# chhylp123/BitMapperBS

Hardware: NVIDIA B200
Metric: mapped_reads_per_sec (higher is better)
Workload: dtype u64

## Files before the change

bitmapperbs_b200/csrc/bmbs_kernels.cuh:

```cuda
#pragma once
#include "bmbs_device.cuh"
#include "bmbs_sort_replay.h"
#include "bmbs_band_walk.h"
#include "../../include/bmbs.h"

namespace bmbs {

constexpr int MAX_TASKS = 28;
constexpr u32 MAX_SEED_HITS = 1000;
constexpr u32 MAX_PE_MULTI = 10000;
constexpr u32 MAX_PE_MULTI_SENSITIVE = 10000;

struct SeedTask { u64 sp; u32 hits; unsigned short mlen, off; };

enum { CNT_HASH = 0, CNT_OCC = 1, CNT_ROWS = 2, CNT_LOCATE_LF = 3, CNT_VERIFIED = 4, CNT_CELLS = 5, CNT_CAND = 6, CNT_WINBYTES = 7 };

struct __align__(16) VerifyItem { u64 site; u32 wi, vote, code_off, L, k, pad; };

struct BatchView {
  const char* ascii; const u64* offsets; int n_reads; int pe;
  u32* codes; uint4* rplanes; u32* len; unsigned short* first_c; unsigned char* kk;
  unsigned char* state; unsigned char* flags;
  short* one_mm; u64* site0;
  u32* list_count;
// ... 40 lines not shown
    const u32 cb = b0 | (b1 << 1) | (bad << 2);
    nib = (cb & 0xFu) | ((cb >> 4) & 0xF0u) | ((cb >> 8) & 0xF00u) | ((cb >> 12) & 0xF000u);
    o.bad = gather4(bad); o.isn = gather4(isn);
  }
  o.nib = nib; o.lo = gather4(b0); o.hi = gather4(b1);
  return o;
}

__device__ __forceinline__ u32 spread8(u32 v) {
  u32 t = (v * 0x1001u) & 0x000F000Fu;
  t = (t * 0x41u) & 0x03030303u;
  return (t * 9u) & 0x11111111u;
}
__device__ __forceinline__ bool pack8(u32 x0, u32 x1, u32& nib, u32& lo8, u32& hi8) {
  const u32 a1 = x0 >> 1, a2 = x0 >> 2, c1 = x1 >> 1, c2 = x1 >> 2;
  const u32 l0 = (a1 ^ a2) & 0x01010101u, h0 = a2 & 0x01010101u, l1 = (c1 ^ c2) & 0x01010101u, h1 = c2 & 0x01010101u;
  lo8 = ((l1 * 16u + l0) * 0x01020408u) >> 24;
  hi8 = ((h1 * 16u + h0) * 0x01020408u) >> 24;
  nib = spread8(hi8) * 2u + spread8(lo8);
  const u32 d0 = x0 ^ __byte_perm(0x54474341u, 0u, nib), d1 = x1 ^ __byte_perm(0x54474341u, 0u, nib >> 16);
  return (d0 | d1) == 0;
}

__global__ void __launch_bounds__(128) pack_reads(BatchView b) {
  const int r = (blockIdx.x * blockDim.x + threadIdx.x) >> 3, sub = threadIdx.x & 7;
  const bool live = r < b.n_reads;
  u64 beg = 0; u32 L = 0;
  if (live) { beg = b.offsets[r]; L = (u32)(b.offsets[r + 1] - beg); }
  u32* w = b.codes + (live ? code_word_offset(b.offsets, r) : 0);
  uint4* pl = b.rplanes + (live ? plane_chunk_offset(b.offsets, r) : 0);
  u32 first_c = L;
  for (u32 c = sub; c * 32 < L; c += 8) {
    const u64 addr = (u64)(b.ascii) + beg + (u64)c * 32;
    const u64* q = (const u64*)(addr & ~7ull);
    const unsigned sh = (unsigned)(addr & 7ull) * 8;
    u64 x[5];
#pragma unroll
    for (int i = 0; i < 5; ++i) x[i] = __ldg(q + i);
    if (sh) {
#pragma unroll
      for (int i = 0; i < 4; ++i) x[i] = (x[i] >> sh) | (x[i + 1] << (64 - sh));
    }
    const u32 left = L - c * 32;
    u32 lo = 0, hi = 0, bad = 0, isn = 0;
    u32 nw[4] = {0u, 0u, 0u, 0u};
#pragma unroll
    for (int i = 0; i < 4; ++i) {
      const u32 base = 8 * i;
      u32 n8, l8, h8;
      if (base < left && pack8((u32)x[i], (u32)(x[i] >> 32), n8, l8, h8)) {
        const u32 nb = left - base;
        if (nb < 8) { n8 &= (1u << (4 * nb)) - 1u; l8 &= (1u << nb) - 1u; h8 &= (1u << nb) - 1u; }
        nw[i] = n8;
        lo |= l8 << base; hi |= h8 << base;
      } else if (base < left) {
        const Packed4 a = pack4((u32)x[i], left - base);
        const Packed4 d = pack4((u32)(x[i] >> 32), left > base + 4 ? left - base - 4 : 0);
        nw[i] = a.nib | (d.nib << 16);
        lo |= (a.lo | (d.lo << 4)) << base; hi |= (a.hi | (d.hi << 4)) << base;
        bad |= (a.bad | (d.bad << 4)) << base; isn |= (a.isn | (d.isn << 4)) << base;
      }
    }
    *reinterpret_cast<uint4*>(w + c * 4) = make_uint4(nw[0], nw[1], nw[2], nw[3]);
    pl[c] = make_uint4(lo, hi, bad, isn);
    const u32 isc = lo & ~hi & ~bad;
    if (isc) first_c = min(first_c, c * 32 + (u32)__ffs(isc) - 1u);
  }
  for (int o = 4; o; o >>= 1) first_c = min(first_c, __shfl_xor_sync(0xffffffffu, first_c, o));
  if (live && sub == 0) {
    b.len[r] = L;
    b.first_c[r] = (unsigned short)first_c;
    u64 k = (u64)(b.e_rate * (double)L);
    b.kk[r] = (unsigned char)(k >= 31 ? 31 : k);
  }
}

struct SeedHit { u64 hits, sp, ep; u32 mlen; bool has_sa; u64 sa; };

constexpr int SEED_BLOCK = 128;
struct ReadPlanes {
  const uint4* p; const uint4* s; u32 ns;
  __device__ __forceinline__ void stage(const uint4* src, u32 L, uint4* smem_col, u32 cap) {
    p = src; s = smem_col;
    ns = (L >> 5) + 2; if (ns > cap) ns = cap;
    for (u32 i = 0; i < ns; ++i) smem_col[i * SEED_BLOCK] = __ldg(src + i);
  }
  __device__ __forceinline__ uint4 chunk(u32 i) const { return i < ns ? s[i * SEED_BLOCK] : __ldg(p + i); }
  __device__ __forceinline__ void window(u32 pos, u32& lo, u32& hi, u32& bad) const {
    const uint4 a = chunk(pos >> 5), c = chunk((pos >> 5) + 1);
    const unsigned s = pos & 31u;
    lo = __funnelshift_r(a.x, c.x, s); hi = __funnelshift_r(a.y, c.y, s); bad = __funnelshift_r(a.z, c.z, s);
  }
};

__device__ __forceinline__ bool key16(const ReadPlanes& rp, const unsigned char* __restrict__ lut, u32 off, u32& key) {
  u32 lo, hi, bad; rp.window(off, lo, hi, bad);
  if (bad & 0xFFFFu) return false;
  const u32 a = (lo & 0xFFFFu) | ((~lo & ~hi) << 16);
  const u32 i0 = (a & 0xFu) | ((a >> 12) & 0xF0u), i1 = ((a >> 4) & 0xFu) | ((a >> 16) & 0xF0u);
  const u32 i2 = ((a >> 8) & 0xFu) | ((a >> 20) & 0xF0u), i3 = ((a >> 12) & 0xFu) | ((a >> 24) & 0xF0u);
  key = (u32)lut[i0] + 81u * (u32)lut[i1] + 6561u * (u32)lut[i2] + 531441u * (u32)lut[i3];
  return true;
}

struct SymbolStream {
  const ReadPlanes& rp; u32 base, lo, hi, bad;
  __device__ __forceinline__ SymbolStream(const ReadPlanes& r, u32 pos, u32 l, u32 h, u32 b) : rp(r), base(pos), lo(l), hi(h), bad(b) {}
  __device__ __forceinline__ int at(u32 pos) {
    if (pos - base >= 32u) { base = pos; rp.window(pos, lo, hi, bad); }
    const unsigned s = pos - base;
    if ((bad >> s) & 1u) return 3;
    const u32 l = (lo >> s) & 1u, h = (hi >> s) & 1u;
    return (int)(l | ((~(l | h) & 1u) << 1));
  }
};

__device__ __forceinline__ bool kmer_ext(const DevIndex& ix, const unsigned char* __restrict__ lut, u32 lo, u32 hi, u32 bad, u32& ext) {
  const u32 mask = (1u << ix.kdepth) - 1u;
  if (bad & mask) return false;
  ext = lut[(lo & mask) | (((~lo & ~hi) & mask) << 4)];
  return true;
}

enum { START_NONE = 0, START_ANSWER = 1, START_LF = 2 };
__device__ __forceinline__ int seed_start(const DevIndex& ix, const ReadPlanes& rp, const unsigned char* lut, u32 off, u32 cur, bool exact,
                                          u32& m, u64& top, u64& bot, bool& one_sa, u32& lo, u32& hi, u32& bad, u32& n_hash) {
  int how = START_LF;
  u32 key;
  one_sa = false;
  if (cur < (exact ? 17u : 18u) || !key16(rp, lut, off, key)) how = START_NONE;
  else {
    m = 16;
    rp.window(off + 16, lo, hi, bad);
    bool in_table = false;
    if (ix.ktab && cur >= 16 + ix.kdepth) {
      u32 ext;
      if (kmer_ext(ix, lut, lo, hi, bad, ext)) {
        const u64 e = __ldg(ix.ktab + (u64)key * ix.kpow + ext); ++n_hash;
        const u64 size = e >> 39; const u32 code = (u32)(e >> 36) & 7u;
        if (size != KTAB_SAT) {
          in_table = true;
          if (code == 0) how = START_NONE;
          else {
            m = 15 + code; top = e & 0xFFFFFFFFFull; bot = top + size; one_sa = size == 1;
            const bool stops_short = m < 16 + ix.kdepth;
            if (!exact) { if (one_sa || stops_short) how = START_ANSWER; }
            else if (stops_short && size >= 2) how = START_NONE;
          }
        }
      }
    }
    if (!in_table) {
      hash_query(ix, key, top, bot); ++n_hash;
      if (bot <= top) how = START_NONE;
    }
  }
  if (how == START_NONE) { m = 0; top = 0; bot = 0; one_sa = false; }
  return how;
}

__device__ __forceinline__ bool exact_tail_matches(const DevIndex& ix, const ReadPlanes& rp, u64 s0, u32 off, u32 from, u32 cur) {
  if (s0 + cur > 2 * ix.N) return false;
  for (u32 p = off + from; p < off + cur; p += 32) {
    u32 rlo, rhi, rbad; rp.window(p, rlo, rhi, rbad);
    const u64 g = s0 + (p - off);
    const uint2 w0 = __ldg(ix.planes + (g >> 5)), w1 = __ldg(ix.planes + (g >> 5) + 1);
    const unsigned sh = (unsigned)g & 31u;
    const u32 glo = __funnelshift_r(w0.x, w1.x, sh), ghi = __funnelshift_r(w0.y, w1.y, sh);
    u32 mism = (rlo ^ glo) | (~rlo & (rhi ^ ghi)) | rbad;
    const u32 left = off + cur - p;
    if (left < 32u) mism &= (1u << left) - 1u;
    if (mism) return false;
  }
  return true;
}

__device__ __forceinline__ SeedHit seed_until_unique(const DevIndex& ix, const ReadPlanes& rp, const unsigned char* lut, u32 off, u32 cur,
                                                     u32& n_occ, u32& n_hash) {
  u32 m = 0, lo = 0, hi = 0, bad = 0; u64 top = 0, bot = 0; bool one_sa = false;
  const int how = seed_start(ix, rp, lut, off, cur, false, m, top, bot, one_sa, lo, hi, bad, n_hash);
  SeedHit h; h.hits = 0; h.sp = 0; h.ep = 0; h.mlen = m; h.has_sa = false; h.sa = 0;
  if (how == START_NONE) return h;
  if (how == START_ANSWER) {
    if (one_sa) { h.hits = 1; h.has_sa = true; h.sa = top; }
    else { h.sp = top; h.ep = bot; h.hits = bot - top; }
    return h;
  }
  u64 ptop = ~0ull, pbot = ~0ull;
  SymbolStream ss(rp, off + 16, lo, hi, bad);
  for (; m < cur; ++m) {
    ptop = top; pbot = bot;
    if (bot - top == 1) break;
    const int c = ss.at(off + m);
    if (c > 2) { bot = top; break; }
    n_occ += lf_pair(ix, top, bot, c);
    if (bot <= top) break;
  }
  h.mlen = m;
  if (bot <= top) { h.sp = ptop; h.ep = pbot; } else { h.sp = top; h.ep = bot; }
  h.hits = h.ep - h.sp;
  return h;
}

__device__ __forceinline__ u64 count_exact(const DevIndex& ix, const ReadPlanes& rp, const unsigned char* lut, u32 off, u32 cur, u64& sp, u64& ep,
                                           bool& have_site, u64& site, u32& n_occ, u32& n_hash, u32& n_rows, u32& n_llf) {
  have_site = false;
  u32 m = 0, lo = 0, hi = 0, bad = 0; u64 top = 0, bot = 0; bool one_sa = false;
  if (seed_start(ix, rp, lut, off, cur, true, m, top, bot, one_sa, lo, hi, bad, n_hash) == START_NONE) return 0;
  const u64 sa_known = top;
  SymbolStream ss(rp, off + 16, lo, hi, bad);
  for (; m < cur; ++m) {
    if (bot <= top) break;
    if (bot - top == 1) {
      int s = 0; const u64 sa = one_sa ? sa_known : locate_row(ix, top, s); n_llf += s; ++n_rows;
      const u64 s0 = 2 * ix.N - sa - m;
      if (!exact_tail_matches(ix, rp, s0, off, m, cur)) return 0;
      have_site = true; site = s0 - off;
      return 1;
    }
    const int c = ss.at(off + m);
    if (c > 2) return 0;
    n_occ += lf_pair(ix, top, bot, c);
  }
  if (one_sa) {
    const u64 s0 = 2 * ix.N - sa_known - m;
    have_site = true; site = s0 - off;
    return 1;
  }
  sp = top; ep = bot;
  return bot <= top ? 0 : bot - top;
}

__device__ __forceinline__ u32 next_offset_unmatched(const ReadPlanes& rp, u32 L, u32 off) {
  if ((int)L - (int)off < 18) return L;
  const uint4 a = rp.chunk(off >> 5), c = rp.chunk((off >> 5) + 1);
  const u32 n8 = __funnelshift_r(a.w, c.w, off & 31u) & 0xFFu;
  return n8 ? off + (u32)__ffs(n8) : off + 8;
}

__device__ __forceinline__ int compare_rest(const DevIndex& ix, const ReadPlanes& rp, u64 site, u32 L, u32& mlen) {
  int errors = 0;
  const bool inside = window_inside(ix, site, L);
  const u32 from = mlen;
  for (u32 c0 = from & ~31u; c0 < L; c0 += 32) {
    const uint4 r = rp.chunk(c0 >> 5);
    u32 mism;
    if (inside) {
      const u64 g = site + c0;
      const uint2 w0 = __ldg(ix.planes + (g >> 5)), w1 = __ldg(ix.planes + (g >> 5) + 1);
      const unsigned sh = (unsigned)g & 31u;
      const u32 glo = __funnelshift_r(w0.x, w1.x, sh), ghi = __funnelshift_r(w0.y, w1.y, sh);
      mism = (((r.x ^ glo) | (r.y ^ ghi)) & ~(r.x & r.y & glo & ~ghi)) | r.z;
    } else mism = 0xFFFFFFFFu;
    if (c0 < from) mism &= ~0u << (from - c0);
    if (L - c0 < 32u) mism &= (1u << (L - c0)) - 1u;
    if (mism) {
      if (errors == 0) { mlen = c0 + (u32)__ffs(mism) - 1u; errors = 1; mism &= mism - 1u; }
      if (mism) { errors = 2; break; }
    }
  }
  return errors;
}

struct SeedCounters { u32 n_occ = 0, n_hash = 0, n_rows = 0, n_llf = 0; };

__device__ __forceinline__ void build_key_lut(unsigned char* lut) {
  for (u32 i = threadIdx.x; i < 256; i += blockDim.x) {
    u32 v = 0, p3 = 1;
    for (u32 t = 0; t < 4; ++t) { v += p3 * (((i >> t) & 1u) | (((i >> (4 + t)) & 1u) << 1)); p3 *= 3; }
    lut[i] = (unsigned char)v;
  }
}

__device__ __forceinline__ void flush_counters(u64* s_cnt, const SeedCounters& c, u64* counters) {
  atomicAdd(&s_cnt[0], (u64)c.n_hash); atomicAdd(&s_cnt[1], (u64)c.n_occ); atomicAdd(&s_cnt[2], (u64)c.n_rows); atomicAdd(&s_cnt[3], (u64)c.n_llf);
  __syncthreads();
  if (threadIdx.x == 0) {
    atomicAdd(counters + CNT_HASH, s_cnt[0]); atomicAdd(counters + CNT_OCC, s_cnt[1]);
    atomicAdd(counters + CNT_ROWS, s_cnt[2]); atomicAdd(counters + CNT_LOCATE_LF, s_cnt[3]);
  }
}

__device__ __forceinline__ void list_append(u32* list, u32* count, bool pred, u32 r) {
  const u32 active = __activemask();
  const u32 m = __ballot_sync(active, pred);
  if (!m) return;
  const int lane = threadIdx.x & 31, leader = __ffs(m) - 1;
  u32 base = 0;
  if (lane == leader) base = atomicAdd(count, (u32)__popc(m));
  base = __shfl_sync(active, base, leader);
  if (pred) list[base + __popc(m & ((1u << lane) - 1u))] = r;
}

struct TaskWriter {
  const BatchView& b; const u32& r; u32& nt; u32& nc;
  __device__ __forceinline__ void emit(u64 a, u32 hits, u32 mlen, u32 o) {
    if (nt < MAX_TASKS) { SeedTask t; t.sp = a; t.hits = hits; t.mlen = (unsigned short)mlen; t.off = (unsigned short)o; b.tasks[(size_t)nt * b.n_reads + r] = t; }
    ++nt; nc += hits ? hits : 1u;
  }
  __device__ __forceinline__ void store() { b.ntask[r] = nt < MAX_TASKS ? nt : MAX_TASKS; b.ncand[r] = nt <= MAX_TASKS ? nc : 0xFFFFFFFFu; }
};

enum { SK_FIRST = 0, SK_SECOND = 1, SK_REST = 2 };
enum { PH_IDLE = 0, PH_REFILL = 1, PH_START = 2, PH_LF = 3, PH_COMPARE = 4, PH_DONE = 5 };

__global__ void __launch_bounds__(128) seed_reads(DevIndex ix, BatchView b, u32 plane_cap) {
  extern __shared__ uint4 s_planes[];
  __shared__ u64 s_cnt[4];
  __shared__ unsigned char s_lut[256];
  if (threadIdx.x < 4) s_cnt[threadIdx.x] = 0;
  build_key_lut(s_lut);
  __syncthreads();
  const int lane = threadIdx.x & 31;
  const u32 n_reads = (u32)b.n_reads;
  SeedCounters cn;
  ReadPlanes rp; rp.p = nullptr; rp.s = s_planes + threadIdx.x; rp.ns = 0;
  int ph = PH_REFILL;
  __shared__ u32 s_w[21][SEED_BLOCK];
  __shared__ u64 s_d[4][SEED_BLOCK];
  const int tx = threadIdx.x;
  u32 &r = s_w[0][tx], &L = s_w[1][tx], &first_c = s_w[2][tx], &off = s_w[3][tx], &first_len = s_w[4][tx], &max_seeds = s_w[5][tx], &seed_id = s_w[6][tx];
  u32 &nt = s_w[7][tx], &nc = s_w[8][tx], &bn = s_w[9][tx], &bs0 = s_w[10][tx], &bs1 = s_w[11][tx], &bep = s_w[12][tx], &bel = s_w[13][tx];
  u32 &first_cands = s_w[14][tx], &g_mlen = s_w[15][tx], &is_multi = s_w[16][tx], &second_ok = s_w[17][tx];
  int &state = reinterpret_cast<int&>(s_w[18][tx]), &get_error = reinterpret_cast<int&>(s_w[19][tx]), &one_mm = reinterpret_cast<int&>(s_w[20][tx]);
  u64 &sp = s_d[0][tx], &ep = s_d[1][tx], &site0 = s_d[2][tx], &g_hits = s_d[3][tx];
  u32 kind = SK_FIRST;
  u32 s_off = 0, s_cur = 0, m = 0;
  u64 top = 0, bot = 0, ptop = 0, pbot = 0, sa_known = 0;
  bool known_sa = false;
  u32 ss_base = 0, ss_lo = 0, ss_hi = 0, ss_bad = 0;
  TaskWriter tw{b, r, nt, nc};
  auto symbol_at = [&](u32 pos) -> int {
    if (pos - ss_base >= 32u) { ss_base = pos; rp.window(pos, ss_lo, ss_hi, ss_bad); }
    const unsigned sh = pos - ss_base;
    const u32 l = (ss_lo >> sh) & 1u, h = (ss_hi >> sh) & 1u, bad = (ss_bad >> sh) & 1u;
    return (int)((l | ((~(l | h) & 1u) << 1)) | (bad * 3u));
  };
  auto finish = [&]() {
    b.state[r] = (unsigned char)state;
    b.flags[r] = (unsigned char)((is_multi ? 1 : 0) | (second_ok ? 2 : 0));
    b.one_mm[r] = (short)one_mm;
    b.site0[r] = site0;
    tw.store();
    if (b.sensitive) {
      const bool resolved = state == BMBS_EXACT_UNIQUE || state == BMBS_MULTI_EXACT;
      unsigned short* k5 = b.bk + (size_t)r * 5;
      k5[0] = (unsigned short)(resolved ? 0 : bn); k5[1] = (unsigned short)bs0; k5[2] = (unsigned short)bs1; k5[3] = (unsigned short)bep;
      k5[4] = (unsigned short)(resolved ? 0 : bel);
      b.first_cands[r] = (unsigned short)(resolved ? 0 : first_cands);
    }
    ph = PH_REFILL;
  };
  auto next_rest = [&]() {
    kind = SK_REST;
    if (seed_id < max_seeds && off < L) { s_off = off; s_cur = L - off; ph = PH_START; } else finish();
  };
  auto first_rest = [&](u32 mlen) {
    one_mm = (int)mlen;
    if (mlen == L && g_hits > 1 && (!b.pe || g_hits <= b.multi_cap)) {
      is_multi = 1;
      if (first_c == L) {
        state = BMBS_MULTI_EXACT;
        if (b.pe) tw.emit(sp, (u32)g_hits, mlen, 0);
        else if (b.amb_out) tw.emit(sp, (u32)(g_hits > MAX_SEED_HITS ? MAX_SEED_HITS : g_hits), mlen, 0);
        finish();
        return;
      }
    }
    if (g_hits != 1 && mlen >= b.seed_len && g_hits <= MAX_SEED_HITS && g_hits != 0) tw.emit(sp, (u32)g_hits, mlen, 0);
    const bool used = g_hits == 1 || (g_mlen >= b.seed_len && g_hits <= MAX_SEED_HITS);
    bn = used ? 1 : 0; bel = used ? first_len : 0; first_cands = nc;
    off = mlen == 0 ? next_offset_unmatched(rp, L, 0) : mlen / 2;
    seed_id = 1;
    if (get_error == 1 && L - first_len >= 17) { kind = SK_SECOND; s_off = first_len; s_cur = L - first_len; ph = PH_START; }
    else next_rest();
  };
  auto second_done = [&]() {
    const u64 hits = known_sa ? 1 : (bot > top ? bot - top : 0);
    if (hits <= MAX_SEED_HITS) {
      if (known_sa) tw.emit(sa_known, 0, 0, 0); else if (hits) tw.emit(top, (u32)hits, s_cur, s_off);
      second_ok = 1; finish();
    } else next_rest();
  };
  auto greedy_done = [&]() {
    const u64 hits = known_sa ? 1 : bot - top;
    const u32 mlen = m;
    if (!known_sa) { sp = top; ep = bot; }
    if (kind == SK_FIRST) {
      g_hits = hits; g_mlen = mlen; first_len = mlen;
      if (hits == 1) ph = PH_COMPARE;
      else first_rest(mlen);
    } else {
      bool used = true;
      if (hits == 1) { if (known_sa) tw.emit(2 * ix.N - sa_known - mlen - off, 0, 0, 0); else tw.emit(sp, 1, mlen, off); }
      else if (mlen >= b.seed_len && hits <= MAX_SEED_HITS) { if (hits) tw.emit(sp, (u32)hits, mlen, off); }
      else { used = false; if (s_cur == mlen) { finish(); return; } }
      if (used) { if (bn == 0) bs0 = off; else if (bn == 1) bs1 = off; bep = bel; bel = off + mlen; ++bn; }
      off = mlen == 0 ? next_offset_unmatched(rp, L, off) : off + mlen / 2;
      ++seed_id;
      next_rest();
    }
  };
  for (;;) {
    const u32 m_lf = __ballot_sync(0xffffffffu, ph == PH_LF), m_cmp = __ballot_sync(0xffffffffu, ph == PH_COMPARE);
    const u32 m_tr = __ballot_sync(0xffffffffu, ph == PH_DONE || ph == PH_START || ph == PH_REFILL);
    if (!(m_lf | m_cmp | m_tr)) break;
    const int c_lf = __popc(m_lf), c_cmp = __popc(m_cmp), c_tr = __popc(m_tr);
    const bool do_tr = c_tr >= c_lf && c_tr >= c_cmp, do_lf = !do_tr && c_lf >= c_cmp;
    if (do_tr) {
      if (ph == PH_DONE) { if (kind == SK_SECOND) second_done(); else greedy_done(); }
      const u32 m_refill = __ballot_sync(0xffffffffu, ph == PH_REFILL);
      const int c_refill = __popc(m_refill);
      if (m_refill) {
      u32 base = 0;
      const int leader = __ffs(m_refill) - 1;
      if (lane == leader) base = atomicAdd(b.list_count, (u32)c_refill);
      base = __shfl_sync(0xffffffffu, base, leader);
      if (ph == PH_REFILL) {
        const u32 i = base + __popc(m_refill & ((1u << lane) - 1u));
        if (i >= n_reads) ph = PH_IDLE;
        else {
          r = i;
          L = b.len[r]; first_c = b.first_c[r];
          rp.stage(b.rplanes + plane_chunk_offset(b.offsets, (int)r), L, s_planes + threadIdx.x, plane_cap);
          { u64 ms = (u64)L / 10 - 1; if (ms > 25) ms = 25; max_seeds = (u32)ms; }
          nt = 0; nc = 0; off = 0; first_len = 0; seed_id = 0; sp = 0; ep = 0; site0 = 0;
          state = BMBS_NONE; get_error = -1; one_mm = 0; is_multi = 0; second_ok = 0;
          bn = 0; bs0 = 0; bs1 = 0; bep = 0; bel = 0; first_cands = 0;
          if (max_seeds > 0 && L > 0) { kind = SK_FIRST; s_off = 0; s_cur = L; ph = PH_START; }
          else finish();
        }
      }
      }
      if (ph == PH_START) {
        const int how = seed_start(ix, rp, s_lut, s_off, s_cur, kind == SK_SECOND, m, top, bot, known_sa, ss_lo, ss_hi, ss_bad, cn.n_hash);
        ss_base = s_off + 16; sa_known = top;
        if (how == START_LF) { ph = PH_LF; ptop = ~0ull; pbot = ~0ull; }
        else ph = PH_DONE;
      }
    } else if (do_lf) {
      if (ph == PH_LF) {
        if (kind != SK_SECOND) {
          bool stop = true;
          if (m < s_cur) {
            ptop = top; pbot = bot;
            const int c = symbol_at(s_off + m);
            if (bot - top != 1) {
              if (c > 2) bot = top;
              else {
                cn.n_occ += lf_pair(ix, top, bot, c);
                if (bot > top) { ++m; stop = m >= s_cur; }
              }
            }
          }
          if (stop) { if (bot <= top) { top = ptop; bot = pbot; } ph = PH_DONE; }
        } else {
          if (m < s_cur && bot > top) {
            if (bot - top == 1) ph = PH_COMPARE;
            else {
              const int c = symbol_at(s_off + m);
              if (c > 2) { bot = top; ph = PH_DONE; }
              else { cn.n_occ += lf_pair(ix, top, bot, c); ++m; }
            }
          } else {
            if (known_sa) sa_known = 2 * ix.N - sa_known - m - s_off;
            ph = PH_DONE;
          }
        }
      }
    } else {
      if (ph == PH_COMPARE) {
        if (kind == SK_FIRST) {
          int st = 0; const u64 sa = known_sa ? sa_known : locate_row(ix, sp, st); cn.n_llf += st; ++cn.n_rows;
          u32 mlen = g_mlen;
          const u64 site = 2 * ix.N - sa - mlen;
          tw.emit(site, 0, 0, 0);
          if (mlen > first_c) mlen = first_c;
          int errors = 0;
          if (mlen != L) errors = compare_rest(ix, rp, site, L, mlen);
          get_error = errors;
          if (errors == 0) { state = BMBS_EXACT_UNIQUE; site0 = site; finish(); }
          else first_rest(mlen);
        } else {
          int st = 0; const u64 sa = known_sa ? sa_known : locate_row(ix, top, st); cn.n_llf += st; ++cn.n_rows;
          const u64 s0 = 2 * ix.N - sa - m;
          known_sa = exact_tail_matches(ix, rp, s0, s_off, m, s_cur); sa_known = s0 - s_off;
          if (!known_sa) bot = top;
          ph = PH_DONE;
        }
      }
    }
  }
  flush_counters(s_cnt, cn, b.counters);
}

constexpr int SEG_CAP = 256;
struct Seg { u64 sp; u32 start; u32 info; };

__global__ void __launch_bounds__(128) expand_locate(DevIndex ix, BatchView b) {
  __shared__ Seg s_seg[4][SEG_CAP];
  __shared__ u64 s_cnt[2];
  if (threadIdx.x < 2) s_cnt[threadIdx.x] = 0;
  __syncthreads();
  const int lane = threadIdx.x & 31;
  Seg* seg = s_seg[threadIdx.x >> 5];
  const int r = blockIdx.x * blockDim.x + threadIdx.x;
  const bool ok = !*b.status, live = ok && r < b.n_reads;
  const u32 nt = live ? b.ntask[r] : 0u;
  const u32 c0 = ok ? b.coff[min(r, b.n_reads)] : 0u, c1 = ok ? b.coff[min(r + 1, b.n_reads)] : 0u;
  u32 incl = nt;
#pragma unroll
  for (int o = 1; o < 32; o <<= 1) { const u32 t = __shfl_up_sync(0xffffffffu, incl, o); if (lane >= o) incl += t; }
  const u32 excl = incl - nt;
  u64 steps = 0, rows = 0;
  int lo_lane = 0;
  while (lo_lane < 32) {
    const u32 base = __shfl_sync(0xffffffffu, excl, lo_lane);
    const bool fits = lane >= lo_lane && incl - base <= (u32)SEG_CAP;
    const int hi_lane = lo_lane + __popc(__ballot_sync(0xffffffffu, fits));
    if (fits) {
      u32 s = c0;
      for (u32 t = 0; t < nt; ++t) {
        const SeedTask k = b.tasks[(size_t)t * b.n_reads + r];
        Seg g; g.sp = k.sp; g.start = s;
        g.info = k.hits ? (u32)k.mlen + (u32)k.off : 0x80000000u;
        seg[excl - base + t] = g;
        s += k.hits ? k.hits : 1u;
      }
    }
    __syncwarp();
    const u32 n_seg = __shfl_sync(0xffffffffu, incl, hi_lane - 1) - base;
    const u32 s_begin = __shfl_sync(0xffffffffu, c0, lo_lane), s_end = __shfl_sync(0xffffffffu, c1, hi_lane - 1);
    if (n_seg) {
      for (u32 s = s_begin + lane; s < s_end; s += 32) {
        u32 lo = 0, hi = n_seg;
        while (hi - lo > 1) { const u32 mid = (lo + hi) >> 1; if (seg[mid].start <= s) lo = mid; else hi = mid; }
        const Seg g = seg[lo];
        u64 site = g.sp;
        if (!(g.info >> 31)) {
          int st; const u64 sa = locate_row(ix, g.sp + (u64)(s - g.start), st);
          site = 2 * ix.N - sa - (u64)(g.info & 0xFFFFu); ++rows; steps += st;
        }
        b.cand[s] = site;
      }
    }
    __syncwarp();
    lo_lane = hi_lane;
  }
  atomicAdd(&s_cnt[0], rows); atomicAdd(&s_cnt[1], steps);
  __syncthreads();
  if (threadIdx.x == 0) { atomicAdd(b.counters + CNT_ROWS, s_cnt[0]); atomicAdd(b.counters + CNT_LOCATE_LF, s_cnt[1]); }
}

__device__ __forceinline__ bool classify_read(BatchView& b, int r, u32 beg, u32 n, bool lane0) {
  if (b.round == 1) { if (n == 0) { if (lane0) b.nv[r] = 0; return false; } return true; }
  const int st = b.state[r];
  if (st == BMBS_EXACT_UNIQUE) { if (lane0) { b.nv[r] = b.pe ? 1u : 0u; if (n) b.vcnt[beg] = 0; } return false; }
  if (st == BMBS_MULTI_EXACT) {
    if (!b.pe) {
      if (lane0) { const u32 keep = b.amb_out ? n : 0u; for (u32 i = 0; i < keep; ++i) b.vcnt[beg + i] = 0; b.nv[r] = keep; }
      return false;
    }
    return true;
  }
  if (n == 0) { if (lane0) b.nv[r] = 0; return false; }
  if ((b.flags[r] & 2) && (n == 1 || (n == 2 && b.cand[beg] == b.cand[beg + 1]))) {
    if (lane0) { b.state[r] = BMBS_ONE_MISMATCH; b.site0[r] = b.cand[beg]; b.nv[r] = b.pe ? 1u : 0u; b.vcnt[beg] = 0; }
    return false;
  }
  if (lane0) b.state[r] = BMBS_VERIFY;
  return true;
}

__device__ __forceinline__ u64 window_start(u64 c, u64 k) { return c < k ? 0ull : c - k; }

template <int N>
__device__ __forceinline__ void sort_regs(u64 (&v)[N]) {
#pragma unroll
  for (int k = 2; k <= N; k <<= 1)
#pragma unroll
    for (int j = k >> 1; j > 0; j >>= 1)
#pragma unroll
      for (int i = 0; i < N; ++i) {
        const int l = i ^ j;
        if (l > i) {
          const u64 a = v[i], c = v[l];
          const bool sw = ((i & k) == 0) ? (a > c) : (a < c);
          v[i] = sw ? c : a; v[l] = sw ? a : c;
        }
      }
}

template <int N>
__device__ __forceinline__ void sort_encode_small(BatchView& b, int r, u32 beg, u32 n, bool live, bool multi) {
  u64 v[N];
#pragma unroll
  for (int i = 0; i < N; ++i) v[i] = (live && (u32)i < n) ? b.cand[beg + i] : ~0ull;
  sort_regs<N>(v);
  if (!live) return;
  if (multi) {
#pragma unroll
    for (int i = 0; i < N; ++i) if ((u32)i < n) { b.cand[beg + i] = v[i]; b.vcnt[beg + i] = 0; }
    b.nv[r] = n;
    return;
  }
  const u64 k = b.kk[r];
  u32 out = 0, run = 0;
#pragma unroll
  for (int i = 0; i < N; ++i) {
    if ((u32)i < n) {
      ++run;
      const bool last = (u32)(i + 1) == n || (i + 1 < N && v[i + 1] != v[i]);
      if (last) { b.cand[beg + out] = window_start(v[i], k); b.vcnt[beg + out] = run; ++out; run = 0; }
    }
  }
  b.nv[r] = out;
}

__global__ void __launch_bounds__(128) votes_classify(BatchView b) {
  const int r = blockIdx.x * blockDim.x + threadIdx.x;
  int which = -1; u32 beg = 0, n = 0;
  if (r < b.n_reads && !*b.status) {
    beg = b.coff[r]; n = b.coff[r + 1] - beg;
    if (classify_read(b, r, beg, n, true)) which = n <= 16 ? 0 : n <= 32 ? 1 : n <= 256 ? 2 : n <= 1024 ? 3 : 4;
  }
  const bool small = which == 0;
  if (__any_sync(0xffffffffu, small)) {
    const bool multi = small && b.round == 0 && b.state[r] == BMBS_MULTI_EXACT;
    if (__all_sync(0xffffffffu, !small || n <= 8)) sort_encode_small<8>(b, r, beg, n, small, multi);
    else sort_encode_small<16>(b, r, beg, n, small, multi);
  }
  list_append(b.sort32, b.sort_count + 1, which == 1, (u32)r);
  list_append(b.mid_list, b.sort_count + 2, which == 2, (u32)r);
  list_append(b.big1k_list, b.sort_count + 3, which == 3, (u32)r);
  list_append(b.big_list, b.big_count, which == 4, (u32)r);
}

template <int W>
__global__ void __launch_bounds__(128) votes_sort(BatchView b) {
  const u32 nlist = *b.status ? 0u : b.sort_count[1];
  const u32* list = b.sort32;
  const int lane = threadIdx.x & 31, sub = lane & (W - 1), half_shift = lane & ~(W - 1);
  const u32 groups = gridDim.x * blockDim.x / W;
  for (u32 g0 = 0; g0 < nlist; g0 += groups) {
    const u32 g = g0 + (blockIdx.x * blockDim.x + threadIdx.x) / W;
    const bool live = g < nlist;
    int r = 0; u32 beg = 0, n = 0;
    if (live) { r = (int)list[g]; beg = b.coff[r]; n = b.coff[r + 1] - beg; }
    u64 v = sub < (int)n ? b.cand[beg + sub] : ~0ull;
#pragma unroll
    for (int k = 2; k <= W; k <<= 1)
#pragma unroll
      for (int j = k >> 1; j > 0; j >>= 1) {
        const u64 o = __shfl_xor_sync(0xffffffffu, v, j);
        const bool take_min = ((sub & k) == 0) == ((sub & j) == 0);
        v = take_min ? (o < v ? o : v) : (o > v ? o : v);
      }
    const bool multi = live && b.round == 0 && b.state[r] == BMBS_MULTI_EXACT;
    const u64 prev = __shfl_up_sync(0xffffffffu, v, 1);
    const bool head = live && !multi && sub < (int)n && (sub == 0 || prev != v);
    const u32 heads = (__ballot_sync(0xffffffffu, head) >> half_shift) & (W == 32 ? 0xffffffffu : 0xffffu);
    if (multi) { if (sub < (int)n) { b.cand[beg + sub] = v; b.vcnt[beg + sub] = 0; } if (sub == 0) b.nv[r] = n; }
    else if (live) {
      if (head) {
        const u32 idx = __popc(heads & ((1u << sub) - 1u));
        const u32 later = heads & ~((2u << sub) - 1u);
        const u32 next = later ? (u32)(__ffs(later) - 1) : n;
        b.cand[beg + idx] = window_start(v, (u64)b.kk[r]);
        b.vcnt[beg + idx] = next - sub;
      }
      if (sub == 0) b.nv[r] = __popc(heads);
    }
  }
}

template <int E, int T>
__device__ __forceinline__ void bitonic_regs(u64 (&v)[E], const int tid, u64* xch) {
#pragma unroll
  for (int k = 2; k <= E * T; k <<= 1) {
    const bool up = ((tid * E) & k) == 0;
#pragma unroll
    for (int j = k >> 1; j > 0; j >>= 1) {
      if (j >= 32 * E) {
        __syncthreads();
#pragma unroll
        for (int i = 0; i < E; ++i) xch[i * T + tid] = v[i];
        __syncthreads();
        const int pt = tid ^ (j / E);
        const bool take_min = up == ((tid & (j / E)) == 0);
#pragma unroll
        for (int i = 0; i < E; ++i) { const u64 o = xch[i * T + pt]; v[i] = take_min ? (o < v[i] ? o : v[i]) : (o > v[i] ? o : v[i]); }
      } else if (j >= E) {
        const bool take_min = up == ((tid & (j / E)) == 0);
#pragma unroll
        for (int i = 0; i < E; ++i) { const u64 o = __shfl_xor_sync(0xffffffffu, v[i], j / E); v[i] = take_min ? (o < v[i] ? o : v[i]) : (o > v[i] ? o : v[i]); }
      } else {
#pragma unroll
        for (int i = 0; i < E; ++i) {
          if ((i & j) == 0) {
            const bool asc = k < E ? ((i & k) == 0) : up;
            const u64 a = v[i], c = v[i | j];
            const bool sw = asc ? (a > c) : (a < c);
            v[i] = sw ? c : a; v[i | j] = sw ? a : c;
          }
        }
      }
    }
  }
}

__device__ __forceinline__ void warp_encode_runs(BatchView& b, int r, u32 beg, u32 n, const u64* a, int lane) {
  const u64 k = b.kk[r];
  u32 base = 0;
  for (u32 c0 = 0; c0 < n; c0 += 32) {
    const u32 i = c0 + lane;
    const bool head = i < n && (i == 0 || a[i - 1] != a[i]);
    const u32 bal = __ballot_sync(0xffffffffu, head);
    if (head) {
      u32 e = i + 1; while (e < n && a[e] == a[i]) ++e;
      const u32 idx = base + __popc(bal & ((1u << lane) - 1u));
      b.cand[beg + idx] = window_start(a[i], k);
      b.vcnt[beg + idx] = e - i;
    }
    base += __popc(bal);
  }
  if (lane == 0) b.nv[r] = base;
}

template <int E>
__device__ __forceinline__ void warp_sort_keys(const u64* __restrict__ src, u32 n, u64* a, int lane) {
  u64 v[E];
#pragma unroll
  for (int i = 0; i < E; ++i) { const u32 e = (u32)lane * E + i; v[i] = e < n ? src[e] : ~0ull; }
  bitonic_regs<E, 32>(v, lane, nullptr);
  __syncwarp();
#pragma unroll
  for (int i = 0; i < E; ++i) a[lane * E + i] = v[i];
  __syncwarp();
}

__global__ void __launch_bounds__(128) votes_mid(BatchView b) {
  __shared__ u64 s_keys[4][32 * 8];
  const u32 nlist = *b.status ? 0u : b.sort_count[2];
  const int lane = threadIdx.x & 31, wid = threadIdx.x >> 5;
  const u32 warps = gridDim.x * (blockDim.x >> 5);
  u64* a = s_keys[wid];
  for (u32 g = blockIdx.x * (blockDim.x >> 5) + wid; g < nlist; g += warps) {
    const int r = (int)b.mid_list[g];
    const u32 beg = b.coff[r], n = b.coff[r + 1] - beg;
    if (n <= 64) warp_sort_keys<2>(b.cand + beg, n, a, lane);
    else if (n <= 128) warp_sort_keys<4>(b.cand + beg, n, a, lane);
    else warp_sort_keys<8>(b.cand + beg, n, a, lane);
    if (b.round == 0 && b.state[r] == BMBS_MULTI_EXACT) {
      for (u32 i = lane; i < n; i += 32) { b.cand[beg + i] = a[i]; b.vcnt[beg + i] = 0; }
      if (lane == 0) b.nv[r] = n;
    } else warp_encode_runs(b, r, beg, n, a, lane);
    __syncwarp();
  }
}

template <int E, int T>
__device__ __forceinline__ void block_sort_keys(const u64* __restrict__ src, u32 n, u64* keys, int tid) {
  u64 v[E];
#pragma unroll
  for (int i = 0; i < E; ++i) { const u32 e = (u32)tid * E + i; v[i] = e < n ? src[e] : ~0ull; }
  bitonic_regs<E, T>(v, tid, keys);
  __syncthreads();
#pragma unroll
  for (int i = 0; i < E; ++i) keys[tid * E + i] = v[i];
  __syncthreads();
}

__global__ void __launch_bounds__(128) votes_big1k(BatchView b) {
  constexpr int T = 128;
  __shared__ u64 s_keys[8 * T];
  const u32 nlist = *b.status ? 0u : b.sort_count[3];
  const int tid = threadIdx.x, lane = tid & 31;
  for (u32 g = blockIdx.x; g < nlist; g += gridDim.x) {
    const int r = (int)b.big1k_list[g];
    const u32 beg = b.coff[r], n = b.coff[r + 1] - beg;
    if (n <= 4 * T) block_sort_keys<4, T>(b.cand + beg, n, s_keys, tid);
    else block_sort_keys<8, T>(b.cand + beg, n, s_keys, tid);
    if (b.round == 0 && b.state[r] == BMBS_MULTI_EXACT) {
      for (u32 i = tid; i < n; i += T) { b.cand[beg + i] = s_keys[i]; b.vcnt[beg + i] = 0; }
      if (tid == 0) b.nv[r] = n;
    } else if (tid < 32) warp_encode_runs(b, r, beg, n, s_keys, lane);
    __syncthreads();
  }
}

constexpr int BIG_SMEM_ELEMS = 16384;
constexpr int BIG_THREADS = 512;
__global__ void __launch_bounds__(BIG_THREADS) votes_big(BatchView b, u32 cap, u32 min_p, u32 max_p) {
  extern __shared__ u64 s_buf[];
// ... 1377 lines not shown
```

Measured before the change: 169.8 million.

## Regroup seed state machine by phase across block via shared-memory masks

```diff
diff --git a/bitmapperbs_b200/csrc/bmbs_kernels.cuh b/bitmapperbs_b200/csrc/bmbs_kernels.cuh
--- a/bitmapperbs_b200/csrc/bmbs_kernels.cuh
+++ b/bitmapperbs_b200/csrc/bmbs_kernels.cuh
@@ -366,178 +366,203 @@
 };
 
 enum { SK_FIRST = 0, SK_SECOND = 1, SK_REST = 2 };
-enum { PH_IDLE = 0, PH_REFILL = 1, PH_START = 2, PH_LF = 3, PH_COMPARE = 4, PH_DONE = 5 };
+enum { PH_LF = 0, PH_DONE = 1, PH_START = 2, PH_LOCATE = 3, PH_COMPARE = 4, PH_REFILL = 5, PH_STAGE = 6, PH_KINDS = 7, PH_IDLE = PH_KINDS };
+constexpr u32 SEED_IDS = 16;
+
+template <class T, class V> struct Narrow {
+  T* p;
+  __device__ __forceinline__ operator V() const { return (V)*p; }
+  __device__ __forceinline__ Narrow& operator=(V v) { *p = (T)v; return *this; }
+  __device__ __forceinline__ Narrow& operator=(const Narrow& o) { *p = (T)(V)o; return *this; }
+  __device__ __forceinline__ Narrow& operator++() { *p = (T)((V)*p + 1); return *this; }
+};
+typedef Narrow<unsigned short, u32> U16;
+typedef Narrow<unsigned char, u32> U8;
+
+__device__ __forceinline__ u32 nth_slot(const u32* mk, u32 j) {
+  u32 w = 0, x = mk[0];
+  while (j >= (u32)__popc(x)) { j -= (u32)__popc(x); x = mk[++w]; }
+  u32 pos = 0;
+#pragma unroll
+  for (u32 h = 16; h; h >>= 1) {
+    const u32 c = (u32)__popc(x & ((1u << h) - 1u));
+    if (j >= c) { j -= c; x >>= h; pos += h; }
+  }
+  return 32 * w + pos;
+}
 
 __global__ void __launch_bounds__(128) seed_reads(DevIndex ix, BatchView b, u32 plane_cap) {
+  constexpr u32 MW = SEED_BLOCK / 32;
   extern __shared__ uint4 s_planes[];
   __shared__ u64 s_cnt[4];
   __shared__ unsigned char s_lut[256];
-  if (threadIdx.x < 4) s_cnt[threadIdx.x] = 0;
+  __shared__ __align__(16) u32 s_mask[3][PH_KINDS][MW];
+  __shared__ u32 s_pool[2][5];
+  __shared__ u32 s_w[7][SEED_BLOCK];
+  __shared__ unsigned short s_h[19][SEED_BLOCK];
+  __shared__ unsigned char s_b[5][SEED_BLOCK];
+  __shared__ u64 s_d[5][SEED_BLOCK];
+  const u32 tx = threadIdx.x;
+  const u32 n_reads = (u32)b.n_reads;
+  if (tx < 4) s_cnt[tx] = 0;
   build_key_lut(s_lut);
+  for (u32 i = tx; i < 3 * PH_KINDS * MW; i += SEED_BLOCK) (&s_mask[0][0][0])[i] = i / MW == PH_REFILL ? ~0u : 0u;
+  if (tx == 0) {
+    const u32 base = atomicAdd(b.list_count, (u32)SEED_BLOCK);
+    s_pool[0][0] = min(base, n_reads); s_pool[0][1] = min(base + SEED_BLOCK, n_reads);
+    s_pool[0][2] = 0; s_pool[0][3] = 0; s_pool[0][4] = base >= n_reads;
+  }
   __syncthreads();
-  const int lane = threadIdx.x & 31;
-  const u32 n_reads = (u32)b.n_reads;
   SeedCounters cn;
-  ReadPlanes rp; rp.p = nullptr; rp.s = s_planes + threadIdx.x; rp.ns = 0;
-  int ph = PH_REFILL;
-  __shared__ u32 s_w[21][SEED_BLOCK];
-  __shared__ u64 s_d[4][SEED_BLOCK];
-  const int tx = threadIdx.x;
-  u32 &r = s_w[0][tx], &L = s_w[1][tx], &first_c = s_w[2][tx], &off = s_w[3][tx], &first_len = s_w[4][tx], &max_seeds = s_w[5][tx], &seed_id = s_w[6][tx];
-  u32 &nt = s_w[7][tx], &nc = s_w[8][tx], &bn = s_w[9][tx], &bs0 = s_w[10][tx], &bs1 = s_w[11][tx], &bep = s_w[12][tx], &bel = s_w[13][tx];
-  u32 &first_cands = s_w[14][tx], &g_mlen = s_w[15][tx], &is_multi = s_w[16][tx], &second_ok = s_w[17][tx];
-  int &state = reinterpret_cast<int&>(s_w[18][tx]), &get_error = reinterpret_cast<int&>(s_w[19][tx]), &one_mm = reinterpret_cast<int&>(s_w[20][tx]);
-  u64 &sp = s_d[0][tx], &ep = s_d[1][tx], &site0 = s_d[2][tx], &g_hits = s_d[3][tx];
-  u32 kind = SK_FIRST;
-  u32 s_off = 0, s_cur = 0, m = 0;
-  u64 top = 0, bot = 0, ptop = 0, pbot = 0, sa_known = 0;
-  bool known_sa = false;
-  u32 ss_base = 0, ss_lo = 0, ss_hi = 0, ss_bad = 0;
-  TaskWriter tw{b, r, nt, nc};
-  auto symbol_at = [&](u32 pos) -> int {
-    if (pos - ss_base >= 32u) { ss_base = pos; rp.window(pos, ss_lo, ss_hi, ss_bad); }
-    const unsigned sh = pos - ss_base;
-    const u32 l = (ss_lo >> sh) & 1u, h = (ss_hi >> sh) & 1u, bad = (ss_bad >> sh) & 1u;
-    return (int)((l | ((~(l | h) & 1u) << 1)) | (bad * 3u));
-  };
-  auto finish = [&]() {
-    b.state[r] = (unsigned char)state;
-    b.flags[r] = (unsigned char)((is_multi ? 1 : 0) | (second_ok ? 2 : 0));
-    b.one_mm[r] = (short)one_mm;
-    b.site0[r] = site0;
-    tw.store();
-    if (b.sensitive) {
-      const bool resolved = state == BMBS_EXACT_UNIQUE || state == BMBS_MULTI_EXACT;
-      unsigned short* k5 = b.bk + (size_t)r * 5;
-      k5[0] = (unsigned short)(resolved ? 0 : bn); k5[1] = (unsigned short)bs0; k5[2] = (unsigned short)bs1; k5[3] = (unsigned short)bep;
-      k5[4] = (unsigned short)(resolved ? 0 : bel);
-      b.first_cands[r] = (unsigned short)(resolved ? 0 : first_cands);
-    }
-    ph = PH_REFILL;
-  };
-  auto next_rest = [&]() {
-    kind = SK_REST;
-    if (seed_id < max_seeds && off < L) { s_off = off; s_cur = L - off; ph = PH_START; } else finish();
-  };
-  auto first_rest = [&](u32 mlen) {
-    one_mm = (int)mlen;
-    if (mlen == L && g_hits > 1 && (!b.pe || g_hits <= b.multi_cap)) {
-      is_multi = 1;
-      if (first_c == L) {
-        state = BMBS_MULTI_EXACT;
-        if (b.pe) tw.emit(sp, (u32)g_hits, mlen, 0);
-        else if (b.amb_out) tw.emit(sp, (u32)(g_hits > MAX_SEED_HITS ? MAX_SEED_HITS : g_hits), mlen, 0);
-        finish();
-        return;
-      }
-    }
-    if (g_hits != 1 && mlen >= b.seed_len && g_hits <= MAX_SEED_HITS && g_hits != 0) tw.emit(sp, (u32)g_hits, mlen, 0);
-    const bool used = g_hits == 1 || (g_mlen >= b.seed_len && g_hits <= MAX_SEED_HITS);
-    bn = used ? 1 : 0; bel = used ? first_len : 0; first_cands = nc;
-    off = mlen == 0 ? next_offset_unmatched(rp, L, 0) : mlen / 2;
-    seed_id = 1;
-    if (get_error == 1 && L - first_len >= 17) { kind = SK_SECOND; s_off = first_len; s_cur = L - first_len; ph = PH_START; }
-    else next_rest();
-  };
-  auto second_done = [&]() {
-    const u64 hits = known_sa ? 1 : (bot > top ? bot - top : 0);
-    if (hits <= MAX_SEED_HITS) {
-      if (known_sa) tw.emit(sa_known, 0, 0, 0); else if (hits) tw.emit(top, (u32)hits, s_cur, s_off);
-      second_ok = 1; finish();
-    } else next_rest();
-  };
-  auto greedy_done = [&]() {
-    const u64 hits = known_sa ? 1 : bot - top;
-    const u32 mlen = m;
-    if (!known_sa) { sp = top; ep = bot; }
-    if (kind == SK_FIRST) {
-      g_hits = hits; g_mlen = mlen; first_len = mlen;
-      if (hits == 1) ph = PH_COMPARE;
-      else first_rest(mlen);
-    } else {
-      bool used = true;
-      if (hits == 1) { if (known_sa) tw.emit(2 * ix.N - sa_known - mlen - off, 0, 0, 0); else tw.emit(sp, 1, mlen, off); }
-      else if (mlen >= b.seed_len && hits <= MAX_SEED_HITS) { if (hits) tw.emit(sp, (u32)hits, mlen, off); }
-      else { used = false; if (s_cur == mlen) { finish(); return; } }
-      if (used) { if (bn == 0) bs0 = off; else if (bn == 1) bs1 = off; bep = bel; bel = off + mlen; ++bn; }
-      off = mlen == 0 ? next_offset_unmatched(rp, L, off) : off + mlen / 2;
-      ++seed_id;
-      next_rest();
-    }
-  };
-  for (;;) {
-    const u32 m_lf = __ballot_sync(0xffffffffu, ph == PH_LF), m_cmp = __ballot_sync(0xffffffffu, ph == PH_COMPARE);
-    const u32 m_tr = __ballot_sync(0xffffffffu, ph == PH_DONE || ph == PH_START || ph == PH_REFILL);
-    if (!(m_lf | m_cmp | m_tr)) break;
-    const int c_lf = __popc(m_lf), c_cmp = __popc(m_cmp), c_tr = __popc(m_tr);
-    const bool do_tr = c_tr >= c_lf && c_tr >= c_cmp, do_lf = !do_tr && c_lf >= c_cmp;
-    if (do_tr) {
-      if (ph == PH_DONE) { if (kind == SK_SECOND) second_done(); else greedy_done(); }
-      const u32 m_refill = __ballot_sync(0xffffffffu, ph == PH_REFILL);
-      const int c_refill = __popc(m_refill);
-      if (m_refill) {
-      u32 base = 0;
-      const int leader = __ffs(m_refill) - 1;
-      if (lane == leader) base = atomicAdd(b.list_count, (u32)c_refill);
-      base = __shfl_sync(0xffffffffu, base, leader);
-      if (ph == PH_REFILL) {
-        const u32 i = base + __popc(m_refill & ((1u << lane) - 1u));
-        if (i >= n_reads) ph = PH_IDLE;
-        else {
-          r = i;
-          L = b.len[r]; first_c = b.first_c[r];
-          rp.stage(b.rplanes + plane_chunk_offset(b.offsets, (int)r), L, s_planes + threadIdx.x, plane_cap);
-          { u64 ms = (u64)L / 10 - 1; if (ms > 25) ms = 25; max_seeds = (u32)ms; }
-          nt = 0; nc = 0; off = 0; first_len = 0; seed_id = 0; sp = 0; ep = 0; site0 = 0;
-          state = BMBS_NONE; get_error = -1; one_mm = 0; is_multi = 0; second_ok = 0;
-          bn = 0; bs0 = 0; bs1 = 0; bep = 0; bel = 0; first_cands = 0;
-          if (max_seeds > 0 && L > 0) { kind = SK_FIRST; s_off = 0; s_cur = L; ph = PH_START; }
-          else finish();
+  for (u32 it = 0;; ++it) {
+    const u32 (*mk)[MW] = s_mask[it % 3];
+    u32 live = 0, ph = PH_IDLE, j = 0, n_refill = 0;
+#pragma unroll
+    for (u32 k = 0; k < PH_KINDS; ++k) {
+      const uint4 w = *reinterpret_cast<const uint4*>(mk[k]);
+      const u32 c = (u32)(__popc(w.x) + __popc(w.y) + __popc(w.z) + __popc(w.w));
+      if (tx - live < c) { ph = k; j = tx - live; }
+      if (k == PH_REFILL) n_refill = c;
+      live += c;
+    }
+    if (live == 0) break;
+    if (tx < PH_KINDS * MW) (&s_mask[(it + 2) % 3][0][0])[tx] = 0u;
+    const u32* P = s_pool[it & 1];
+    u32* Q = s_pool[(it + 1) & 1];
+    bool grab = false; u32 grabbed = 0;
+    if (tx == 0) {
+      u32 c0 = P[0], c1 = P[1], n0 = P[2], n1 = P[3];
+      const u32 a = min(n_refill, c1 - c0);
+      c0 += a; n0 += min(n_refill - a, n1 - n0);
+      if (c0 == c1) { c0 = n0; c1 = n1; n0 = n1; }
+      Q[0] = c0; Q[1] = c1; Q[2] = n0; Q[3] = n1; Q[4] = P[4];
+      grab = n0 == n1 && !P[4];
+      if (grab) grabbed = atomicAdd(b.list_count, SEED_IDS);
+    }
+    if (ph != PH_IDLE) {
+      const u32 sl = nth_slot(mk[ph], j);
+      u32 &r = s_w[0][sl], &nt = s_w[1][sl], &nc = s_w[2][sl], &pc = s_w[3][sl];
+      u32 &ss_lo = s_w[4][sl], &ss_hi = s_w[5][sl], &ss_bad = s_w[6][sl];
+      U16 L{&s_h[0][sl]}, first_c{&s_h[1][sl]}, off{&s_h[2][sl]}, first_len{&s_h[3][sl]}, max_seeds{&s_h[4][sl]}, seed_id{&s_h[5][sl]};
+      U16 bn{&s_h[6][sl]}, bs0{&s_h[7][sl]}, bs1{&s_h[8][sl]}, bep{&s_h[9][sl]}, bel{&s_h[10][sl]}, first_cands{&s_h[11][sl]}, g_mlen{&s_h[12][sl]};
+      U16 s_off{&s_h[13][sl]}, s_cur{&s_h[14][sl]}, m{&s_h[15][sl]}, ss_base{&s_h[16][sl]};
+      Narrow<short, int> get_error{(short*)&s_h[17][sl]}, one_mm{(short*)&s_h[18][sl]};
+      U8 kind{&s_b[0][sl]}, known_sa{&s_b[1][sl]}, is_multi{&s_b[2][sl]}, second_ok{&s_b[3][sl]};
+      Narrow<unsigned char, int> state{&s_b[4][sl]};
+      u64 &sp = s_d[0][sl], &g_hits = s_d[1][sl], &top = s_d[2][sl], &bot = s_d[3][sl], &sa_known = s_d[4][sl];
+      u64 site0 = 0;
+      ReadPlanes rp; rp.p = b.rplanes + pc; rp.s = s_planes + sl; rp.ns = min(((u32)L >> 5) + 2, plane_cap);
+      TaskWriter tw{b, r, nt, nc};
+      auto finish = [&]() {
+        b.state[r] = (unsigned char)state;
+        b.flags[r] = (unsigned char)((is_multi ? 1 : 0) | (second_ok ? 2 : 0));
+        b.one_mm[r] = (short)one_mm;
+        b.site0[r] = site0;
+        tw.store();
+        if (b.sensitive) {
+          const bool resolved = state == BMBS_EXACT_UNIQUE || state == BMBS_MULTI_EXACT;
+          unsigned short* k5 = b.bk + (size_t)r * 5;
+          k5[0] = (unsigned short)(resolved ? 0 : bn); k5[1] = (unsigned short)bs0; k5[2] = (unsigned short)bs1; k5[3] = (unsigned short)bep;
+          k5[4] = (unsigned short)(resolved ? 0 : bel);
+          b.first_cands[r] = (unsigned short)(resolved ? 0 : first_cands);
         }
-      }
-      }
-      if (ph == PH_START) {
-        const int how = seed_start(ix, rp, s_lut, s_off, s_cur, kind == SK_SECOND, m, top, bot, known_sa, ss_lo, ss_hi, ss_bad, cn.n_hash);
-        ss_base = s_off + 16; sa_known = top;
-        if (how == START_LF) { ph = PH_LF; ptop = ~0ull; pbot = ~0ull; }
-        else ph = PH_DONE;
-      }
-    } else if (do_lf) {
+        ph = PH_REFILL;
+      };
+      auto next_rest = [&]() {
+        kind = SK_REST;
+        if (seed_id < max_seeds && off < L) { s_off = off; s_cur = L - off; ph = PH_START; } else finish();
+      };
+      auto first_rest = [&](u32 mlen) {
+        one_mm = (int)mlen;
+        if (mlen == L && g_hits > 1 && (!b.pe || g_hits <= b.multi_cap)) {
+          is_multi = 1;
+          if (first_c == L) {
+            state = BMBS_MULTI_EXACT;
+            if (b.pe) tw.emit(sp, (u32)g_hits, mlen, 0);
+            else if (b.amb_out) tw.emit(sp, (u32)(g_hits > MAX_SEED_HITS ? MAX_SEED_HITS : g_hits), mlen, 0);
+            finish();
+            return;
+          }
+        }
+        if (g_hits != 1 && mlen >= b.seed_len && g_hits <= MAX_SEED_HITS && g_hits != 0) tw.emit(sp, (u32)g_hits, mlen, 0);
+        const bool used = g_hits == 1 || (g_mlen >= b.seed_len && g_hits <= MAX_SEED_HITS);
+        bn = used ? 1 : 0; bel = used ? first_len : 0; first_cands = nc;
+        off = mlen == 0 ? next_offset_unmatched(rp, L, 0) : mlen / 2;
+        seed_id = 1;
+        if (get_error == 1 && L - first_len >= 17) { kind = SK_SECOND; s_off = first_len; s_cur = L - first_len; ph = PH_START; }
+        else next_rest();
+      };
+      auto second_done = [&]() {
+        const u64 hits = known_sa ? 1 : (bot > top ? bot - top : 0);
+        if (hits <= MAX_SEED_HITS) {
+          if (known_sa) tw.emit(sa_known, 0, 0, 0); else if (hits) tw.emit(top, (u32)hits, s_cur, s_off);
+          second_ok = 1; finish();
+        } else next_rest();
+      };
+      auto greedy_done = [&]() {
+        const u64 hits = known_sa ? 1 : bot - top;
+        const u32 mlen = m;
+        if (!known_sa) sp = top;
+        if (kind == SK_FIRST) {
+          g_hits = hits; g_mlen = mlen; first_len = mlen;
+          if (hits == 1) ph = known_sa ? PH_COMPARE : PH_LOCATE;
+          else first_rest(mlen);
+        } else {
+          bool used = true;
+          if (hits == 1) { if (known_sa) tw.emit(2 * ix.N - sa_known - mlen - off, 0, 0, 0); else tw.emit(sp, 1, mlen, off); }
+          else if (mlen >= b.seed_len && hits <= MAX_SEED_HITS) { if (hits) tw.emit(sp, (u32)hits, mlen, off); }
+          else { used = false; if (s_cur == mlen) { finish(); return; } }
+          if (used) { if (bn == 0) bs0 = off; else if (bn == 1) bs1 = off; bep = bel; bel = off + mlen; ++bn; }
+          off = mlen == 0 ? next_offset_unmatched(rp, L, off) : off + mlen / 2;
+          ++seed_id;
+          next_rest();
+        }
+      };
       if (ph == PH_LF) {
+        u64 t = top, e = bot; u32 mm = m, base = ss_base, lo = ss_lo, hi = ss_hi, bad = ss_bad;
+        const u32 so = s_off, sc = s_cur;
+        auto symbol_at = [&](u32 pos) -> int {
+          if (pos - base >= 32u) { base = pos; rp.window(pos, lo, hi, bad); }
+          const unsigned sh = pos - base;
+          const u32 l = (lo >> sh) & 1u, h = (hi >> sh) & 1u, bd = (bad >> sh) & 1u;
+          return (int)((l | ((~(l | h) & 1u) << 1)) | (bd * 3u));
+        };
         if (kind != SK_SECOND) {
+          const u64 ptop = t, pbot = e;
           bool stop = true;
-          if (m < s_cur) {
-            ptop = top; pbot = bot;
-            const int c = symbol_at(s_off + m);
-            if (bot - top != 1) {
-              if (c > 2) bot = top;
+          if (mm < sc) {
+            const int c = symbol_at(so + mm);
+            if (e - t != 1) {
+              if (c > 2) e = t;
               else {
-                cn.n_occ += lf_pair(ix, top, bot, c);
-                if (bot > top) { ++m; stop = m >= s_cur; }
+                cn.n_occ += lf_pair(ix, t, e, c);
+                if (e > t) { ++mm; stop = mm >= sc; }
               }
             }
           }
-          if (stop) { if (bot <= top) { top = ptop; bot = pbot; } ph = PH_DONE; }
+          if (stop) { if (e <= t) { t = ptop; e = pbot; } ph = PH_DONE; }
         } else {
-          if (m < s_cur && bot > top) {
-            if (bot - top == 1) ph = PH_COMPARE;
+          if (mm < sc && e > t) {
+            if (e - t == 1) ph = known_sa ? PH_COMPARE : PH_LOCATE;
             else {
-              const int c = symbol_at(s_off + m);
-              if (c > 2) { bot = top; ph = PH_DONE; }
-              else { cn.n_occ += lf_pair(ix, top, bot, c); ++m; }
+              const int c = symbol_at(so + mm);
+              if (c > 2) { e = t; ph = PH_DONE; }
+              else { cn.n_occ += lf_pair(ix, t, e, c); ++mm; }
             }
           } else {
-            if (known_sa) sa_known = 2 * ix.N - sa_known - m - s_off;
+            if (known_sa) sa_known = 2 * ix.N - sa_known - mm - so;
             ph = PH_DONE;
           }
         }
-      }
-    } else {
-      if (ph == PH_COMPARE) {
+        top = t; bot = e; m = mm; ss_base = base; ss_lo = lo; ss_hi = hi; ss_bad = bad;
+      } else if (ph == PH_LOCATE) {
+        int st = 0; sa_known = locate_row(ix, top, st); cn.n_llf += st;
+        ph = PH_COMPARE;
+      } else if (ph == PH_COMPARE) {
+        ++cn.n_rows;
         if (kind == SK_FIRST) {
-          int st = 0; const u64 sa = known_sa ? sa_known : locate_row(ix, sp, st); cn.n_llf += st; ++cn.n_rows;
           u32 mlen = g_mlen;
-          const u64 site = 2 * ix.N - sa - mlen;
+          const u64 site = 2 * ix.N - sa_known - mlen;
           tw.emit(site, 0, 0, 0);
           if (mlen > first_c) mlen = first_c;
           int errors = 0;
@@ -546,14 +571,44 @@
           if (errors == 0) { state = BMBS_EXACT_UNIQUE; site0 = site; finish(); }
           else first_rest(mlen);
         } else {
-          int st = 0; const u64 sa = known_sa ? sa_known : locate_row(ix, top, st); cn.n_llf += st; ++cn.n_rows;
-          const u64 s0 = 2 * ix.N - sa - m;
-          known_sa = exact_tail_matches(ix, rp, s0, s_off, m, s_cur); sa_known = s0 - s_off;
-          if (!known_sa) bot = top;
+          const u64 s0 = 2 * ix.N - sa_known - m;
+          const bool hit = exact_tail_matches(ix, rp, s0, s_off, m, s_cur);
+          known_sa = hit; sa_known = s0 - s_off;
+          if (!hit) bot = top;
           ph = PH_DONE;
         }
-      }
-    }
+      } else if (ph == PH_REFILL) {
+        const u32 held = P[1] - P[0];
+        if (j < held + (P[3] - P[2])) {
+          r = j < held ? P[0] + j : P[2] + (j - held);
+          L = b.len[r]; first_c = b.first_c[r]; pc = plane_chunk_offset(b.offsets, (int)r);
+          ph = PH_STAGE;
+        } else if (P[4]) ph = PH_IDLE;
+      } else if (ph == PH_STAGE) {
+        rp.stage(rp.p, L, s_planes + sl, plane_cap);
+        { u64 ms = (u64)L / 10 - 1; if (ms > 25) ms = 25; max_seeds = (u32)ms; }
+        nt = 0; nc = 0; off = 0; first_len = 0; seed_id = 0; sp = 0;
+        state = BMBS_NONE; get_error = -1; one_mm = 0; is_multi = 0; second_ok = 0;
+        bn = 0; bs0 = 0; bs1 = 0; bep = 0; bel = 0; first_cands = 0;
+        if (max_seeds > 0 && L > 0) { kind = SK_FIRST; s_off = 0; s_cur = L; ph = PH_START; }
+        else finish();
+      } else {
+        if (ph == PH_DONE) { if (kind == SK_SECOND) second_done(); else greedy_done(); }
+        if (ph == PH_START) {
+          u32 mm = 0, lo = 0, hi = 0, bad = 0; u64 t = 0, e = 0; bool one = false;
+          const int how = seed_start(ix, rp, s_lut, s_off, s_cur, kind == SK_SECOND, mm, t, e, one, lo, hi, bad, cn.n_hash);
+          m = mm; top = t; bot = e; known_sa = one; sa_known = t;
+          ss_base = s_off + 16; ss_lo = lo; ss_hi = hi; ss_bad = bad;
+          ph = how == START_LF ? PH_LF : PH_DONE;
+        }
+      }
+      if (ph != PH_IDLE) atomicOr(&s_mask[(it + 1) % 3][ph][sl >> 5], 1u << (sl & 31u));
+    }
+    if (grab) {
+      if (grabbed >= n_reads) Q[4] = 1;
+      else { Q[2] = grabbed; Q[3] = min(grabbed + SEED_IDS, n_reads); }
+    }
+    __syncthreads();
   }
   flush_counters(s_cnt, cn, b.counters);
 }
```

Result: slower. 129.1 million (median of 6 runs) (-24.0%).
